# microsoft/DirectXTex

Measured on AMD Instinct MI355X. Metric: Mtexels/s BC7 encode (4096^2 RGBA8, TEX_COMPRESS_DEFAULT), higher is better.
Workload: dtype fp32 seed fit + i32 exact error sums (u8 texels in, 128-bit blocks out); 1 GPU; cfg2: 4096x4096 RGBA8 -> BC7_UNORM, TEX_COMPRESS_DEFAULT, one image per GPU, source and payload resident in HBM (dxtex_compress_device)

## Files before the change

directxtex_amd/csrc/bc6h_encode.hip:

```cpp
#include "dxtex_kernels.h"
#include "bc67_tables.h"
#include "bc7_core.h"
#include "bc6h_core.h"
#include "search_common.h"
#include <algorithm>
#include <cstdlib>
#include <cstdio>
#include <vector>

namespace dxtex
{
namespace
{
using namespace bc6h;

struct Ep16 { uint32_t a01, a2b0, b12; };
__device__ __forceinline__ Ep16 pack_ep16(const int (&A)[3], const int (&B)[3])
{
    Ep16 e;
    e.a01 = (uint32_t(A[0]) & 0xFFFFu) | (uint32_t(A[1]) << 16);
    e.a2b0 = (uint32_t(A[2]) & 0xFFFFu) | (uint32_t(B[0]) << 16);
    e.b12 = (uint32_t(B[1]) & 0xFFFFu) | (uint32_t(B[2]) << 16);
    return e;
}
// ... 1043 lines not shown
}

hipError_t launch_bc6h_encode(const SrcView& src, uint8_t* dst, uint64_t dstRowPitch, bool isSigned, void* scratch,
                              hipStream_t stream, KernelMarks* marks, const SideStreams* side)
{
    BcImage one; one.src = src; one.dst = dst; one.dstRowPitch = dstRowPitch;
    return launch_bc6h_encode_many(&one, 1, isSigned, scratch, stream, marks, side);
}

hipError_t launch_bc6h_encode_many(const BcImage* images, size_t count, bool isSigned, void* scratch, hipStream_t stream, KernelMarks* marks,
                                   const SideStreams* side)
{
#define DXTEX_MARK(NAME) do { if (marks) marks->mark(NAME); } while (0)
    std::vector<BcSeg> segs;
    std::vector<BcPass> passes;
    uint64_t perPass = 0;
    if (!build_passes(images, count, kMaxBlocksPerPass6, segs, passes, &perPass)) return hipSuccess;
    const Scratch6 L(perPass);
    uint8_t* base = static_cast<uint8_t*>(scratch);
    BcSeg* dSegs = reinterpret_cast<BcSeg*>(base + L.total);
    const hipError_t ce = upload_segments(dSegs, segs, passes, stream);
    if (ce != hipSuccess) return ce;
    for (const BcPass& pass : passes)
    {
        Bc6hArgs a;
        set_pass(a.seg, dSegs, segs, pass);
        a.nblocks = pass.nblocks;
        a.isSigned = isSigned ? 1 : 0;
        static const bool noPrune = dev_env("DXTEX_BC6H_NO_PRUNE") != nullptr;
        a.prune = noPrune ? 0 : 1;
        a.fpix = reinterpret_cast<float*>(base + L.fpix);
        a.lists = base + L.lists;
        a.seeds = reinterpret_cast<int*>(base + L.seeds);
        a.recs = reinterpret_cast<Rec6*>(base + L.recs);
        a.orgs = reinterpret_cast<OrgSave*>(base + L.orgs);
        a.order = reinterpret_cast<uint2*>(base + L.order);
        a.tinfo = reinterpret_cast<uint32_t*>(base + L.tinfo);
        a.counters = reinterpret_cast<uint32_t*>(base + L.counters);
        a.best = reinterpret_cast<Best6*>(base + L.best);
        a.bounds = reinterpret_cast<float*>(base + L.bounds);
        a.opts = reinterpret_cast<OptSave*>(base + L.opts);
        a.saveOpt = 0;
        a.boundsReady = 0;
        a.filterStats = 0;
        a.mode = ModeRt();

        DXTEX_MARK("bc6h_rough");
        hipLaunchKernelGGL(bc6h_rough_kernel, dim3((a.nblocks + 3) / 4), dim3(256), 0, stream, a);
        DXTEX_MARK("bc6h_block_seed");
        hipLaunchKernelGGL(bc6h_block_seed_kernel, dim3((a.nblocks + 255) / 256), dim3(256), 0, stream, a);
        if (dev_env("DXTEX_BC6H_DUMP"))
        {
            (void)hipStreamSynchronize(stream);
            const uint32_t n = std::min<uint32_t>(a.nblocks, 4);
            std::vector<uint8_t> l(n * 8); std::vector<int> sd(n * SEED_INTS);
            (void)hipMemcpy(l.data(), a.lists, l.size(), hipMemcpyDeviceToHost);
            (void)hipMemcpy(sd.data(), a.seeds, sd.size() * 4, hipMemcpyDeviceToHost);
            for (uint32_t b = 0; b < n; ++b)
            {
                fprintf(stderr, "block %u shapes:", b);
                for (int i = 0; i < 8; ++i) fprintf(stderr, " %d", l[b * 8 + i]);
                fprintf(stderr, "\n  seeds rank0:");
                for (int i = 0; i < 12; ++i) fprintf(stderr, " %d", sd[b * SEED_INTS + i]);
                fprintf(stderr, "\n");
            }
        }
        static const int onlyMode = dev_env("DXTEX_BC6H_ONLY_MODE") ? atoi(dev_env("DXTEX_BC6H_ONLY_MODE")) : -1;
        static const bool noSearch = dev_env("DXTEX_BC6H_NO_SEARCH") != nullptr;
        static const Bc6hMode kModes[14] = {
            { 0x00, 1, 1, 3, { 10, 10, 10 }, { 5, 5, 5 } }, { 0x01, 1, 1, 3, { 7, 7, 7 }, { 6, 6, 6 } }, { 0x02, 1, 1, 3, { 11, 11, 11 }, { 5, 4, 4 } },
            { 0x06, 1, 1, 3, { 11, 11, 11 }, { 4, 5, 4 } }, { 0x0a, 1, 1, 3, { 11, 11, 11 }, { 4, 4, 5 } }, { 0x0e, 1, 1, 3, { 9, 9, 9 }, { 5, 5, 5 } },
            { 0x12, 1, 1, 3, { 8, 8, 8 }, { 6, 5, 5 } }, { 0x16, 1, 1, 3, { 8, 8, 8 }, { 5, 6, 5 } }, { 0x1a, 1, 1, 3, { 8, 8, 8 }, { 5, 5, 6 } },
            { 0x1e, 1, 0, 3, { 6, 6, 6 }, { 6, 6, 6 } }, { 0x03, 0, 0, 4, { 10, 10, 10 }, { 10, 10, 10 } }, { 0x07, 0, 1, 4, { 11, 11, 11 }, { 9, 9, 9 } },
            { 0x0b, 0, 1, 4, { 12, 12, 12 }, { 8, 8, 8 } }, { 0x0f, 0, 1, 4, { 16, 16, 16 }, { 4, 4, 4 } } };
        auto set_mode_on = [&](Bc6hArgs& a, int mi)
        {
            const Bc6hMode& k = kModes[mi];
            a.mode.index = mi; a.mode.code = k.code; a.mode.regions2 = k.regions2; a.mode.transformed = k.transformed; a.mode.prec = k.prec[0];
            for (int c = 0; c < 3; ++c) a.mode.delta[c] = k.delta[c];
        };
        auto set_mode = [&](int mi) { set_mode_on(a, mi); };
        auto sort_tasks = [&](const Bc6hArgs& a, uint32_t ntasks, hipStream_t stream)
        {
            const uint32_t binGroups = std::min<uint32_t>(kBinGroups, (ntasks + 255) / 256);
            (void)hipMemsetAsync(a.counters, 0, 128 * sizeof(uint32_t), stream);
            hipLaunchKernelGGL(bc7_bin_count_kernel, dim3(binGroups), dim3(256), 0, stream, a.tinfo, ntasks, a.counters);
            hipLaunchKernelGGL(bc7_bin_scan_kernel, dim3(1), dim3(1), 0, stream, a.counters);
            hipLaunchKernelGGL(bc7_bin_scatter_kernel, dim3(binGroups), dim3(256), 0, stream, a.tinfo, ntasks, a.counters, a.order);
        };
        a.taskBase = 0;
        for (int m = 0; m < 4; ++m) a.prec1[m] = kModes[10 + m].prec[0];
        static const std::vector<int> order6 = []
        {
            std::vector<int> o;
            const char* e = dev_env("DXTEX_BC6H_ORDER");
            const char* p = e ? e : DXTEX_BC6H_DEFAULT_ORDER;
            while (*p) { if (*p >= '0' && *p <= '9') o.push_back(int(strtol(p, const_cast<char**>(&p), 10))); else ++p; }
            return o;
        }();
        int prevPrec = -1;
        a.samePrec = 0;
        std::vector<int> run2;
        for (int mi : order6) if (mi >= 0 && mi <= 9 && (onlyMode < 0 || mi == onlyMode)) run2.push_back(mi);
        static const int forkBack = dev_env("DXTEX_BC6H_FORK_BACK") ? atoi(dev_env("DXTEX_BC6H_FORK_BACK")) : 2;
        const SideStreams* fork = (marks || forkBack <= 0 || run2.size() < size_t(forkBack) + 1 || onlyMode >= 0) ? nullptr : side;
        Bc6hArgs a1 = a;
        a1.recs = reinterpret_cast<Rec6*>(base + L.recs1);
        a1.orgs = reinterpret_cast<OrgSave*>(base + L.orgs1);
        a1.order = reinterpret_cast<uint2*>(base + L.order1);
        a1.tinfo = reinterpret_cast<uint32_t*>(base + L.tinfo1);
        a1.counters = reinterpret_cast<uint32_t*>(base + L.counters1);
        a1.samePrec = 0;
        auto one_region_search = [&](hipStream_t stream, KernelMarks* marks)
        {
            const uint32_t gridPP = (a1.nblocks + 255) / 256;
            DXTEX_MARK("bc6h_pre_1region");
            a1.boundsReady = 0;
            for (int m = 0; m < 4; ++m)
            {
                if (onlyMode >= 0 && 10 + m != onlyMode) continue;
                set_mode_on(a1, 10 + m); a1.taskBase = uint32_t(m) * a1.nblocks;
                hipLaunchKernelGGL(bc6h_pre_kernel<0>, dim3(gridPP), dim3(256), 0, stream, a1);
                a1.boundsReady = 1;
            }
            const uint32_t ntasks = a1.nblocks * 4u;
            if (onlyMode >= 0)
                for (int m = 0; m < 4; ++m) if (10 + m != onlyMode) (void)hipMemsetAsync(a1.tinfo + uint64_t(m) * a1.nblocks, 0, uint64_t(a1.nblocks) * 4, stream);
            DXTEX_MARK("bc6h_bin_1region");
            sort_tasks(a1, ntasks, stream);
            DXTEX_MARK("bc6h_perturb_1region");
            static const uint32_t waveMax = dev_env("DXTEX_BC6H_WAVE_MAX") ? uint32_t(strtoul(dev_env("DXTEX_BC6H_WAVE_MAX"), nullptr, 0)) : kWaveTaskMax6;
            if (!noSearch)
            {
                hipLaunchKernelGGL(bc6h_perturb_kernel<16>, dim3(std::min<uint32_t>(kSearchWaves, (ntasks + 63) / 64)), dim3(64), 0, stream, a1, waveMax);
                hipLaunchKernelGGL(bc6h_perturb_wave_kernel, dim3(std::min<uint32_t>(kSearchWaves, ntasks)), dim3(64), 0, stream, a1, waveMax);
            }
        };
        bool forked = false;
        for (size_t at = 0; at < run2.size(); ++at)
        {
            const int mi = run2[at];
            if (fork && at + size_t(forkBack) == run2.size())
            {
                (void)hipEventRecord(fork->forked, stream);
                (void)hipStreamWaitEvent(fork->side[0], fork->forked, 0);
                one_region_search(fork->side[0], nullptr);
                (void)hipEventRecord(fork->joined[0], fork->side[0]);
                forked = true;
            }
            set_mode(mi);
            static const bool noReuse = dev_env("DXTEX_BC6H_NO_REUSE") != nullptr;
            a.samePrec = (!noReuse && prevPrec == kModes[mi].prec[0]) ? 1 : 0;
            prevPrec = kModes[mi].prec[0];
            a.saveOpt = (!noReuse && at + 1 < run2.size() && kModes[run2[at + 1]].prec[0] == kModes[mi].prec[0]) ? 1 : 0;
            const uint32_t ntasks = a.nblocks * 16u;
            const uint32_t gridPP = (a.nblocks + 15) / 16;
            static const char* const kPre[10] = { "bc6h_pre_m0", "bc6h_pre_m1", "bc6h_pre_m2", "bc6h_pre_m3", "bc6h_pre_m4", "bc6h_pre_m5", "bc6h_pre_m6", "bc6h_pre_m7", "bc6h_pre_m8", "bc6h_pre_m9" };
            static const char* const kPerturb[10] = { "bc6h_perturb_m0", "bc6h_perturb_m1", "bc6h_perturb_m2", "bc6h_perturb_m3", "bc6h_perturb_m4", "bc6h_perturb_m5", "bc6h_perturb_m6", "bc6h_perturb_m7", "bc6h_perturb_m8", "bc6h_perturb_m9" };
            static const char* const kPost[10] = { "bc6h_post_m0", "bc6h_post_m1", "bc6h_post_m2", "bc6h_post_m3", "bc6h_post_m4", "bc6h_post_m5", "bc6h_post_m6", "bc6h_post_m7", "bc6h_post_m8", "bc6h_post_m9" };
            DXTEX_MARK(kPre[mi]);
            hipLaunchKernelGGL(bc6h_pre_kernel<1>, dim3(gridPP), dim3(256), 0, stream, a);
            a.boundsReady = 1;
            DXTEX_MARK("bc6h_bin_2region");
            sort_tasks(a, ntasks, stream);
#if defined(DXTEX_DEV)
            static const bool stats6 = dev_env("DXTEX_BC6H_STATS") != nullptr;
            a.filterStats = stats6 ? 1 : 0;
            if (stats6)
            {
                uint32_t c[40] = {};
                (void)hipStreamSynchronize(stream);
// ... 57 lines not shown
```

directxtex_amd/csrc/bc7_encode.hip:

```cpp
#include "dxtex_kernels.h"
#include "bc67_tables.h"
#include "bc7_core.h"
#include "search_common.h"
#include <algorithm>
#include <cstdio>
#include <cstdlib>
#include <vector>

namespace dxtex
{
namespace
{
using namespace bc7;

struct Cand { uint32_t err; uint32_t ord; uint64_t lo, hi; };

enum : int { SLOT_M0 = 0, SLOT_M1, SLOT_M2, SLOT_M3, SLOT_M4A, SLOT_M4B, SLOT_M5, SLOT_M6, SLOT_M7, NUM_SLOTS };
enum : int { LIST_BYTES = 64 };

enum : int { PHASE_ALL = 0, PHASE_EARLY = 1, PHASE_LATE = 2 };

struct Bc7Args
{
    SegTable seg;
// ... 308 lines not shown
    if (a.gate && *a.gate < a.gateMin) return;
    const uint32_t blk = uint32_t(lane) / TM::TPB, r = uint32_t(lane) % TM::TPB;
    const uint32_t nb = nbFirst + blk;
    uint32_t shape, mask, anchor, rot;
    const bool active = (blk < uint32_t(BPW)) && task_geometry<MODE, IM>(a, nb, r, shape, mask, anchor, rot);
    TaskRec rec; rec.A = 0; rec.B = 0; rec.err = 0; rec.orgErr = 0;
    uint32_t npLive = 0;
    if (!__any(active))
    {
        if (nb < a.nblocks && blk < uint32_t(BPW))
        {
            a.recs[uint64_t(nb) * TM::TPB + r] = rec;
            a.tinfo[uint64_t(nb) * TM::TPB + r] = 0;
        }
        return;
    }
    stage_packed<BPW>(a, nbFirst, lane, sL[wave]);
    int lb = 0;
    if (active)
    {
        SubsetResult res; int np; Region rg; Block16 b16;
        task_org<MODE, IM>(nullptr, &sL[wave][blk * 16], mask, anchor, rot, res, np, true, rg, b16,
                           (TM::NS == 2) ? a.seeds + uint64_t(nb) * 64 + (TM::LIST ? 32 : 0) + r
                                         : (TM::NS == 1) ? a.seeds1 + uint64_t(nb) * 2 : a.seeds3 + uint64_t(nb) * 192 + shape * 3 + (r % TM::G));
        rec.A = res.orgA; rec.B = res.orgB; rec.err = res.orgErr; rec.orgErr = res.orgErr;
        npLive = (res.orgErr != 0) ? uint32_t(np) : 0u;
        if (a.prune && npLive)
        {
            lb = subset_lower_bound(&sL[wave][blk * 16], mask, rot, (MODE >= 6) ? 4 : 3);
            if (MODE == 4 || MODE == 5)
            {
                if (rot != 0 || lst_has_alpha(a, nb))
                    lb += scalar_kmeans_lower_bound<(MODE == 4 && IM == 0) ? 8 : 4>(&sL[wave][blk * 16], rot);
            }
            if (MODE < 4)
            {
                const uint32_t* pix = &sL[wave][blk * 16];
#pragma unroll
                for (int i = 0; i < 16; ++i) if ((mask >> i) & 1u) { const int da = 255 - int(pix[i] >> 24); lb += da * da; }
            }
        }
    }
    if (a.prune)
    {
        int candOrg = active ? rec.err : 0, candLb = lb;
#pragma unroll
        for (int d = 1; d < TM::G; d <<= 1) { candOrg += __shfl_xor(candOrg, d); candLb += __shfl_xor(candLb, d); }
        int table = active ? candOrg : 0x7FFFFFFF;
#pragma unroll
        for (int d = TM::G; d < TM::TPB && d < 64; d <<= 1) table = min(table, __shfl_xor(table, d));
        if (nb < a.nblocks && blk < uint32_t(BPW)) table = min(table, a.bestErr[nb]);
        if (candLb > table) npLive = 0;
    }
    if (nb < a.nblocks && blk < uint32_t(BPW))
    {
        a.recs[uint64_t(nb) * TM::TPB + r] = rec;
        a.tinfo[uint64_t(nb) * TM::TPB + r] = (mask & 0xFFFFu) | (rot << 16) | (npLive << 24);
    }
}

template<int MODE, int IM>
__device__ __forceinline__ void search_pickup(const Bc7Args& a, uint2 task, uint32_t* slotCol, SlotRegion& rg)
{
    typedef TaskMap<MODE, IM> TM;
    const uint32_t nb = task.x / TM::TPB;
    const uint32_t mask = task.y & 0xFFFFu, rot = (task.y >> 16) & 3u;
    const uint4* px4 = reinterpret_cast<const uint4*>(a.px + uint64_t(nb) * 16);
    const uint4 q0 = px4[0], q1 = px4[1], q2 = px4[2], q3 = px4[3];
    const uint32_t px[16] = { q0.x, q0.y, q0.z, q0.w, q1.x, q1.y, q1.z, q1.w, q2.x, q2.y, q2.z, q2.w, q3.x, q3.y, q3.z, q3.w };
    int np = 0;
    if (TM::NS == 1)
    {
#pragma unroll
        for (int i = 0; i < 16; ++i) slotCol[i * kSlotStride] = rotate_pixel(px[i], rot);
        np = 16;
    }
    else
    {
#pragma unroll
        for (int i = 0; i < 16; ++i)
            if ((mask >> i) & 1u) { slotCol[np * kSlotStride] = px[i]; ++np; }
    }
    rg.base = slotCol; rg.np = np; rg.p2sum = 0;
}

__device__ __forceinline__ int lanes_below(unsigned long long mask)
{
    return int(__builtin_amdgcn_mbcnt_hi(uint32_t(mask >> 32), __builtin_amdgcn_mbcnt_lo(uint32_t(mask), 0u)));
}

#if defined(DXTEX_BC7_WAVETIMES)
enum : int { WT_KINDS = 3, WT_KEYS = WT_KINDS * 8 * 2 * 3, WT_FIELDS = 6 };
__device__ unsigned long long g_wt[WT_KEYS][8192][WT_FIELDS];
__device__ unsigned int g_wtHist[WT_KEYS][256];
#define WT_BEGIN(KIND) const int wtKey = (((KIND) * 8 + MODE) * 2 + IM) * 3 + CHSET; const bool wtOn = a.phase != PHASE_EARLY; \
    const unsigned long long wt0 = wall_clock64(); unsigned long long wtDr = 0, wtRounds = 0, wtLanes = 0, wtTasks = 0; int wtMine = 0
#define WT_TAKE(IDX) do { wtTasks += (unsigned long long)__popcll(__ballot((IDX) != 0xFFFFFFFFu)); if (!wtDr && q.drained) wtDr = wall_clock64(); } while (0)
#define WT_ROUND(BUSYL) do { ++wtRounds; wtLanes += (unsigned long long)__popcll(__ballot(BUSYL)); if (BUSYL) ++wtMine; } while (0)
#define WT_DONE() do { wtMine = 0; } while (0)
#define WT_END() do { if (wtOn && lane == 0 && wtRounds) { unsigned long long* w_ = g_wt[wtKey][blockIdx.x & 8191]; w_[0] = wt0; w_[1] = wtDr ? wtDr : wall_clock64(); \
    w_[2] = wall_clock64(); w_[3] = wtRounds; w_[4] = wtLanes; w_[5] = wtTasks; } } while (0)
#else
#define WT_BEGIN(KIND) do { } while (0)
#define WT_TAKE(IDX) do { } while (0)
#define WT_ROUND(BUSYL) do { } while (0)
#define WT_DONE() do { } while (0)
#define WT_END() do { } while (0)
#endif
#if !defined(DXTEX_FLAT_SKIP)
#define DXTEX_FLAT_SKIP 1
#endif
template<int MODE, int IM, int CHSET>
constexpr bool kFlatSkip = DXTEX_FLAT_SKIP != 0 && MODE == 6 && CHSET == CH_ALL;

template<int MODE, int IM, int CHSET>
__global__ void __launch_bounds__(64) bc7_perturb_kernel(Bc7Args a, int loop)
{
    typedef LoopCfg<MODE, IM, CHSET> C;
    __shared__ uint32_t sSlot[16 * kSlotStride];
    const int lane = threadIdx.x;
    const uint32_t live = a.counters[34];
    if (live == 0) return;
    if (TaskMap<MODE, IM>::NS == 1 && live <= a.perturbWaveMax) return;
    uint32_t* head = a.counters + kQueueBase + loop;
    uint32_t* slotCol = &sSlot[lane];
    WT_BEGIN(0);

    PerturbState st = perturb_begin<MODE, IM, CHSET>(0, 0, 0);
    SlotRegion rg; rg.base = slotCol; rg.np = 0; rg.p2sum = 0;
    int base = 0;
    uint32_t myTask = 0xFFFFFFFFu;
    uint32_t flatMask = 0, flatVals = 0;
    WaveQueue q; q.lo = q.hi = 0; q.drained = false;
    for (;;)
    {
        const unsigned long long idle = __ballot(myTask == 0xFFFFFFFFu);
        if (idle && !(q.drained && q.lo >= q.hi))
        {
            const uint32_t idx = queue_take(q, head, live, idle, lane);
            WT_TAKE(idx);
            if (idx != 0xFFFFFFFFu)
            {
                const uint2 task = a.order[idx];
                myTask = task.x;
                const TaskRec r = a.recs[myTask];
                search_pickup<MODE, IM>(a, task, slotCol, rg);
                st = perturb_begin<MODE, IM, CHSET>(r.A, r.B, r.err);
                int other;
                base = loop_base<MODE, IM, CHSET>(rg, st.optA, st.optB, &other);
                if (loop_is_settled<CHSET>(r.err, other)) myTask = 0xFFFFFFFFu;
                if constexpr (kFlatSkip<MODE, IM, CHSET>) flatMask = flat_channels(rg, flatVals);
            }
        }
        if constexpr (kFlatSkip<MODE, IM, CHSET>)
        {
            const bool fc = myTask != 0xFFFFFFFFu && flat_call<MODE, IM, CHSET>(st, flatMask, flatVals);
            if (__any(fc))
            {
                const int nearest = eval_nearest<MODE, IM, CHSET>(rg, st, base);
                if (fc && nearest == st.optErr)
                {
                    st = skip_flat_calls<MODE, IM, CHSET>(st);
                    if (st.ch >= C::CH1)
                    {
                        TaskRec* r = a.recs + myTask;
                        r->A = st.optA; r->B = st.optB; r->err = st.optErr;
                        myTask = 0xFFFFFFFFu;
                        WT_DONE();
                    }
                }
            }
// ... 777 lines not shown
    uint64_t lo = 0, hi = 0;
#pragma unroll
    for (int s = 0; s < NUM_SLOTS; ++s)
    {
        if (!((slotMask >> s) & 1u)) continue;
        if (s == SLOT_M7 && a.flagged[1] == 0) continue;
        const Cand v = c[s];
        if (v.err == 0xFFFFFFFFu) continue;
        const uint64_t key = (uint64_t(v.err) << 32) | v.ord;
        if (key < bestKey) { bestKey = key; lo = v.lo; hi = v.hi; }
    }
    const BcSeg& sg = seg_of(a.seg, nb);
    const uint32_t gb = sg.nb0 + (nb - sg.l0);
    const uint32_t by = gb / sg.nbw, bx = gb - by * sg.nbw;
    uint64_t* out = reinterpret_cast<uint64_t*>(sg.dst + uint64_t(by) * sg.dstRowPitch) + 2 * uint64_t(bx);
    out[0] = lo; out[1] = hi;
}
}

namespace
{
const uint64_t kMaxBlocksPerPass = dev_env("DXTEX_MAX_BLOCKS_PER_PASS") ? std::max<uint64_t>(1, strtoull(dev_env("DXTEX_MAX_BLOCKS_PER_PASS"), nullptr, 10)) : (1u << 22);
constexpr int kMaxTasksPerBlock = 64;
const uint64_t kSmallPassBlocks = dev_env("DXTEX_BC7_SMALL_BLOCKS") ? strtoull(dev_env("DXTEX_BC7_SMALL_BLOCKS"), nullptr, 10) : 262144;
struct ScratchLayout
{
    size_t lists, cands, px, recs, order, tinfo, counters, zeroOrd, bestErr, seeds, seeds1, seeds3, flagcnt, auxRecs, auxOrder, auxTinfo, auxCounters, total;
    size_t auxTpb, auxSlices;
    explicit ScratchLayout(uint64_t nb, bool threeSubsets)
    {
        auto up = [](size_t v) { return (v + 255) & ~size_t(255); };
        const size_t tpb = threeSubsets ? kMaxTasksPerBlock : 32;
        const bool small = nb <= kSmallPassBlocks;
        auxTpb = small ? tpb : 4; auxSlices = small ? size_t(kSideStreams) : 2;
        size_t o = 0;
        lists = o; o = up(o + nb * LIST_BYTES);
        cands = o; o = up(o + nb * NUM_SLOTS * sizeof(Cand));
        px = o; o = up(o + nb * 64);
        recs = o; o = up(o + nb * tpb * sizeof(TaskRec));
        order = o; o = up(o + nb * tpb * sizeof(uint2));
        tinfo = o; o = up(o + nb * tpb * sizeof(uint32_t));
        counters = o; o = up(o + 64 * sizeof(uint32_t));
        zeroOrd = o; o = up(o + nb * sizeof(uint32_t));
        bestErr = o; o = up(o + nb * sizeof(int));
        seeds = o; o = up(o + nb * 64 * sizeof(uint2));
        seeds1 = o; o = up(o + nb * 2 * sizeof(uint2));
        seeds3 = o; o = up(o + (threeSubsets ? nb * 192 * sizeof(uint2) : 0));
        flagcnt = o; o = up(o + 256);
        auxRecs = o; o = up(o + auxSlices * nb * auxTpb * sizeof(TaskRec));
        auxOrder = o; o = up(o + auxSlices * nb * auxTpb * sizeof(uint2));
        auxTinfo = o; o = up(o + auxSlices * nb * auxTpb * sizeof(uint32_t));
        auxCounters = o; o = up(o + size_t(kSideStreams) * 64 * sizeof(uint32_t));
        total = o;
    }
};

template<int MODE, int IM>
void launch_mode(const Bc7Args& a0, hipStream_t stream, KernelMarks* marks, const char* const (&names)[7])
{
    typedef TaskMap<MODE, IM> TM;
    constexpr int BPW = (TM::TPB >= 64) ? 1 : 64 / TM::TPB;
    const uint32_t nb = a0.nblocks;
    const uint32_t ntasks = nb * uint32_t(TM::TPB);
    const uint32_t gridPP = (nb + 4 * BPW - 1) / (4 * BPW);
    constexpr bool kWhole = TM::NS == 1;
    constexpr uint32_t kExhMax = (MODE == 6) ? kWaveTaskMax : kWaveTaskMax45;
    static const bool noGroup = dev_env("DXTEX_BC7_NO_GROUP") != nullptr;
    const bool maybeShortP = kWhole && !noGroup && (MODE == 6 || ntasks <= 4u * kPerturbWaveMax);
    const bool maybeShortE = kWhole && !noGroup && (MODE == 6 || ntasks <= 4u * kExhMax);
    const uint32_t wavesP = std::min<uint32_t>(kSearchWaves, (ntasks + 1) / 2), wavesE = std::min<uint32_t>(kSearchWaves, ntasks);
    Bc7Args a = a0;
    a.gate = nullptr; a.gateMin = 0;
    if (a0.flagged && !(a0.flags & BCF_BC7_QUICK))
    {
        if (MODE == 7) { a.gate = a0.flagged + 1; a.gateMin = 1; }
        else if (a0.phase == PHASE_EARLY && (MODE == 4 || MODE == 5)) { a.gate = a0.flagged + 1; a.gateMin = std::max<uint32_t>(1u, a0.earlyAlphaMin); }
        else if (a0.phase == PHASE_EARLY && MODE == 6) { a.gate = a0.flagged; a.gateMin = std::max<uint32_t>(1u, a0.early6Min); }
    }
    a.perturbWaveMax = maybeShortP ? kPerturbWaveMax : 0u;
    a.exhWaveMax = maybeShortE ? kExhMax : 0u;
    if (marks) marks->mark(names[0]);
    hipLaunchKernelGGL((bc7_pre_kernel<MODE, IM>), dim3(gridPP), dim3(256), 0, stream, a);
    if (marks) marks->mark(names[1]);
    (void)hipMemsetAsync(a.counters, 0, 64 * sizeof(uint32_t), stream);
    const uint32_t binGroups = std::min<uint32_t>(kBinGroups, (ntasks + 255) / 256);
    hipLaunchKernelGGL(bc7_bin_count_kernel, dim3(binGroups), dim3(256), 0, stream, a.tinfo, ntasks, a.counters, a.gate, a.gateMin);
    hipLaunchKernelGGL(bc7_bin_scan_kernel, dim3(1), dim3(1), 0, stream, a.counters);
    hipLaunchKernelGGL(bc7_bin_scatter_kernel, dim3(binGroups), dim3(256), 0, stream, a.tinfo, ntasks, a.counters, a.order, a.gate, a.gateMin);
    if (marks) marks->mark(names[2]);
    const uint32_t waves = std::min<uint32_t>(kSearchWaves, (ntasks + 63) / 64);
    static const int tailBelow = dev_env("DXTEX_BC7_TAIL_BELOW") ? atoi(dev_env("DXTEX_BC7_TAIL_BELOW")) : 48;
    static const bool perturbPlain = dev_env("DXTEX_BC7_PERTURB_PLAIN") != nullptr;
    static const int rangeTests = dev_env("DXTEX_BC7_NO_PEEL") ? 3 : ((dev_env("DXTEX_BC7_RANGE_TESTS") ? atoi(dev_env("DXTEX_BC7_RANGE_TESTS")) & 0xFF : DXTEX_RANGE_TESTS) |
                                                                       ((dev_env("DXTEX_BC7_PEEL_LAYERS") ? atoi(dev_env("DXTEX_BC7_PEEL_LAYERS")) : 1) << 8));
    if constexpr (PaletteBits<MODE, IM>::AB == 0)
    {
        if constexpr (MODE == 1 || MODE == 6)
        {
            if (perturbPlain) hipLaunchKernelGGL((bc7_perturb_kernel<MODE, IM, CH_ALL>), dim3(waves), dim3(64), 0, stream, a, 0);
            else hipLaunchKernelGGL((bc7_perturb_filter_kernel<MODE, IM, CH_ALL>), dim3(waves), dim3(64), 0, stream, a, 0);
        }
        else
            hipLaunchKernelGGL((bc7_perturb_kernel<MODE, IM, CH_ALL>), dim3(waves), dim3(64), 0, stream, a, 0);
        if constexpr (kWhole) { if (maybeShortP) hipLaunchKernelGGL((bc7_perturb_wave_kernel<MODE, IM, CH_ALL>), dim3(wavesP), dim3(64), 0, stream, a); }
        if (marks) marks->mark(names[4]);
        if constexpr (kWhole) { if (maybeShortE) hipLaunchKernelGGL((bc7_exhaustive_wave_kernel<MODE, IM, CH_ALL>), dim3(wavesE), dim3(64), 0, stream, a); }
        hipLaunchKernelGGL((bc7_exhaustive_kernel<MODE, IM, CH_ALL>), dim3(waves), dim3(64), 0, stream, a, 1, tailBelow, rangeTests);
    }
    else
    {
        if constexpr (MODE == 4 && IM == 1 && DXTEX_PF_M4 != 0)
        {
            if (perturbPlain) hipLaunchKernelGGL((bc7_perturb_kernel<MODE, IM, CH_COLOR>), dim3(waves), dim3(64), 0, stream, a, 0);
            else hipLaunchKernelGGL((bc7_perturb_filter_kernel<MODE, IM, CH_COLOR>), dim3(waves), dim3(64), 0, stream, a, 0);
        }
        else
            hipLaunchKernelGGL((bc7_perturb_kernel<MODE, IM, CH_COLOR>), dim3(waves), dim3(64), 0, stream, a, 0);
        if (maybeShortP) hipLaunchKernelGGL((bc7_perturb_wave_kernel<MODE, IM, CH_COLOR>), dim3(wavesP), dim3(64), 0, stream, a);
        if (marks) marks->mark(names[3]);
        hipLaunchKernelGGL((bc7_perturb_kernel<MODE, IM, CH_ALPHA>), dim3(waves), dim3(64), 0, stream, a, 1);
        if (maybeShortP) hipLaunchKernelGGL((bc7_perturb_wave_kernel<MODE, IM, CH_ALPHA>), dim3(wavesP), dim3(64), 0, stream, a);
        if (marks) marks->mark(names[4]);
        if (maybeShortE) hipLaunchKernelGGL((bc7_exhaustive_wave_kernel<MODE, IM, CH_COLOR>), dim3(wavesE), dim3(64), 0, stream, a);
        hipLaunchKernelGGL((bc7_exhaustive_kernel<MODE, IM, CH_COLOR>), dim3(waves), dim3(64), 0, stream, a, 2, tailBelow, rangeTests);
        if (marks) marks->mark(names[5]);
        if (maybeShortE) hipLaunchKernelGGL((bc7_exhaustive_wave_kernel<MODE, IM, CH_ALPHA>), dim3(wavesE), dim3(64), 0, stream, a);
        hipLaunchKernelGGL((bc7_exhaustive_kernel<MODE, IM, CH_ALPHA>), dim3(waves), dim3(64), 0, stream, a, 3, tailBelow, rangeTests);
    }
    if (marks) marks->mark(names[6]);
    hipLaunchKernelGGL((bc7_post_kernel<MODE, IM>), dim3(gridPP), dim3(256), 0, stream, a);
#if defined(DXTEX_DEV)
    static const bool stats = dev_env("DXTEX_BC7_STATS") != nullptr;
    if (stats)
    {
        uint32_t c[40] = {};
        (void)hipStreamSynchronize(stream);
        (void)hipMemcpy(c, a.counters, sizeof(c), hipMemcpyDeviceToHost);
        std::fprintf(stderr, "bc7 stats %-22s phase %d: %9u task slots, %9u live; by size 16..1:", names[0], a.phase, ntasks, c[34]);
        for (int b = 16; b >= 1; --b) std::fprintf(stderr, " %u", c[b]);
        std::fprintf(stderr, "\n");
    }
#endif
}
}

#if defined(DXTEX_BC7_WAVETIMES)
namespace
{
void bc7_wavetimes_report()
{
    (void)hipDeviceSynchronize();
    static int call = 0;
    static const int wanted = dev_env("DXTEX_BC7_WT_CALL") ? atoi(dev_env("DXTEX_BC7_WT_CALL")) : 2;
    const bool print = call++ == wanted;
    static std::vector<unsigned long long> h(size_t(WT_KEYS) * 8192 * WT_FIELDS);
    static std::vector<unsigned int> hist(size_t(WT_KEYS) * 256);
    (void)hipMemcpyFromSymbol(h.data(), HIP_SYMBOL(g_wt), h.size() * 8);
    (void)hipMemcpyFromSymbol(hist.data(), HIP_SYMBOL(g_wtHist), hist.size() * 4);
    unsigned long long tAll = ~0ull;
    for (size_t i = 0; i < size_t(WT_KEYS) * 8192; ++i) if (h[i * WT_FIELDS + 2]) tAll = std::min(tAll, h[i * WT_FIELDS]);
    static const char* const kinds[3] = { "perturb", "perturb_filter", "exhaustive" };
    for (int key = 0; key < WT_KEYS; ++key)
    {
        const unsigned long long* w = h.data() + size_t(key) * 8192 * WT_FIELDS;
        std::vector<unsigned long long> st, dr, en; unsigned long long rounds = 0, lanes = 0, life = 0, maxR = 0, tasks = 0, maxT = 0;
        for (int i = 0; i < 8192; ++i)
            if (w[i * WT_FIELDS + 2])
            {
                st.push_back(w[i * WT_FIELDS]); dr.push_back(w[i * WT_FIELDS + 1]); en.push_back(w[i * WT_FIELDS + 2]);
                rounds += w[i * WT_FIELDS + 3]; lanes += w[i * WT_FIELDS + 4]; tasks += w[i * WT_FIELDS + 5];
                life += w[i * WT_FIELDS + 2] - w[i * WT_FIELDS]; maxR = std::max(maxR, w[i * WT_FIELDS + 3]); maxT = std::max(maxT, w[i * WT_FIELDS + 5]);
// ... 246 lines not shown
```

directxtex_amd/csrc/search_common.h:

```cpp
#pragma once
#include <hip/hip_runtime.h>
#include <stdint.h>
#include <algorithm>
#include <cstring>
#include <vector>
#include "dxtex_kernels.h"

namespace dxtex
{
namespace
{
struct BcSeg
{
    SrcView src;
    uint8_t* dst;
    uint64_t dstRowPitch;
    uint32_t nbw;
    uint32_t nb0;
    uint32_t l0;
    uint32_t pad;
};

struct SegTable
{
// ... 40 lines not shown

inline hipError_t upload_segments(BcSeg* dSegs, std::vector<BcSeg>& segs, const std::vector<BcPass>& passes, hipStream_t stream)
{
    bool needTable = false;
    for (const BcPass& pass : passes) needTable |= pass.nseg > 2;
    if (!needTable) return hipSuccess;
    struct Staging { void* host = nullptr; size_t capacity = 0; hipEvent_t consumed = nullptr; bool pending = false; int device = -1; };
    static thread_local Staging st;
    int device = 0;
    hipError_t e = hipGetDevice(&device);
    if (e != hipSuccess) return e;
    if (st.pending) { e = hipEventSynchronize(st.consumed); if (e != hipSuccess) return e; st.pending = false; }
    const size_t bytes = segs.size() * sizeof(BcSeg);
    if (st.device != device || st.capacity < bytes)
    {
        if (st.host) (void)hipHostFree(st.host);
        if (st.consumed) (void)hipEventDestroy(st.consumed);
        st = Staging();
        e = hipHostMalloc(&st.host, std::max<size_t>(bytes, 4096), hipHostMallocDefault);
        if (e != hipSuccess) return e;
        e = hipEventCreateWithFlags(&st.consumed, hipEventDisableTiming);
        if (e != hipSuccess) return e;
        st.capacity = std::max<size_t>(bytes, 4096); st.device = device;
    }
    std::memcpy(st.host, segs.data(), bytes);
    e = hipMemcpyAsync(dSegs, st.host, bytes, hipMemcpyHostToDevice, stream);
    if (e != hipSuccess) return e;
    e = hipEventRecord(st.consumed, stream);
    st.pending = (e == hipSuccess);
    return e;
}

inline void set_pass(SegTable& t, const BcSeg* dSegs, const std::vector<BcSeg>& segs, const BcPass& pass)
{
    t.segs = dSegs + pass.seg0; t.nseg = pass.nseg;
    t.inl[0] = segs[pass.seg0]; t.inl[1] = segs[pass.seg0 + (pass.nseg > 1 ? 1 : 0)];
}

inline size_t seg_table_bytes(uint64_t nblocks, uint64_t maxPerPass, size_t nimages)
{
    const uint64_t perPass = nblocks < maxPerPass ? nblocks : maxPerPass;
    const uint64_t passes = perPass ? (nblocks + perPass - 1) / perPass : 1;
    return ((nimages + passes + 1) * sizeof(BcSeg) + 255) & ~size_t(255);
}

__device__ __forceinline__ void wave_lds_sync()
{
    __builtin_amdgcn_fence(__ATOMIC_RELEASE, "wavefront");
    __builtin_amdgcn_wave_barrier();
    __builtin_amdgcn_fence(__ATOMIC_ACQUIRE, "wavefront");
}

__device__ __forceinline__ int wave_prefix_min(int v)
{
    v = min(v, __builtin_amdgcn_update_dpp(v, v, 0x111, 0xF, 0xF, false));
    v = min(v, __builtin_amdgcn_update_dpp(v, v, 0x112, 0xF, 0xF, false));
    v = min(v, __builtin_amdgcn_update_dpp(v, v, 0x114, 0xF, 0xF, false));
    v = min(v, __builtin_amdgcn_update_dpp(v, v, 0x118, 0xF, 0xF, false));
    v = min(v, __builtin_amdgcn_update_dpp(v, v, 0x142, 0xA, 0xF, false));
    v = min(v, __builtin_amdgcn_update_dpp(v, v, 0x143, 0xC, 0xF, false));
    return v;
}

__device__ __forceinline__ void selection_pass(int& e, uint32_t& s, int lane, int i)
{
    const int v = (lane >= i) ? e : 0x7FFFFFFF;
    const int incl = wave_prefix_min(v);
    int excl = __builtin_amdgcn_update_dpp(0x7FFFFFFF, incl, 0x138, 0xF, 0xF, false);
    if (lane <= i) excl = 0x7FFFFFFF;
    const bool isrec = (lane > i) && (e < excl);
    const unsigned long long mask = __ballot(isrec);
    int srcLane = lane;
    if (isrec)
    {
        const unsigned long long below = mask & ((1ull << lane) - 1ull);
        srcLane = below ? (63 - __clzll(below)) : i;
    }
    else if (lane == i && mask)
        srcLane = 63 - __clzll(mask);
    e = __shfl(e, srcLane);
    s = uint32_t(__shfl(int(s), srcLane));
}

constexpr int kBinGroups = 2048;

__global__ void __launch_bounds__(256) bc7_bin_count_kernel(const uint32_t* tinfo, uint32_t ntasks, uint32_t* counters, const uint32_t* gate = nullptr, uint32_t gateMin = 0)
{
    if (gate && *gate < gateMin) return;
    __shared__ uint32_t hist[17];
    if (threadIdx.x < 17) hist[threadIdx.x] = 0;
    __syncthreads();
    const uint32_t per = (ntasks + gridDim.x - 1) / gridDim.x;
    const uint32_t t0 = blockIdx.x * per, t1 = min(ntasks, t0 + per);
    for (uint32_t t = t0 + threadIdx.x; t < t1; t += 256)
    {
        const uint32_t np = tinfo[t] >> 24;
        if (np) atomicAdd(&hist[np], 1u);
    }
    __syncthreads();
    if (threadIdx.x >= 1 && threadIdx.x <= 16 && hist[threadIdx.x]) atomicAdd(&counters[threadIdx.x], hist[threadIdx.x]);
}

__global__ void bc7_bin_scan_kernel(uint32_t* counters)
{
    if (threadIdx.x != 0 || blockIdx.x != 0) return;
    uint32_t run = 0;
    for (int b = 16; b >= 1; --b) { counters[17 + b] = run; run += counters[b]; }
    counters[34] = run;
}

__global__ void __launch_bounds__(256) bc7_bin_scatter_kernel(const uint32_t* tinfo, uint32_t ntasks, uint32_t* counters, uint2* order, const uint32_t* gate = nullptr, uint32_t gateMin = 0)
{
    if (gate && *gate < gateMin) return;
    __shared__ uint32_t hist[17], cursor[17];
    if (threadIdx.x < 17) hist[threadIdx.x] = 0;
    __syncthreads();
    const uint32_t per = (ntasks + gridDim.x - 1) / gridDim.x;
    const uint32_t t0 = blockIdx.x * per, t1 = min(ntasks, t0 + per);
    for (uint32_t t = t0 + threadIdx.x; t < t1; t += 256)
    {
        const uint32_t np = tinfo[t] >> 24;
        if (np) atomicAdd(&hist[np], 1u);
    }
    __syncthreads();
    if (threadIdx.x >= 1 && threadIdx.x <= 16)
        cursor[threadIdx.x] = hist[threadIdx.x] ? atomicAdd(&counters[17 + threadIdx.x], hist[threadIdx.x]) : 0u;
    __syncthreads();
    for (uint32_t t = t0 + threadIdx.x; t < t1; t += 256)
    {
        const uint32_t ti = tinfo[t], np = ti >> 24;
        if (np) order[atomicAdd(&cursor[np], 1u)] = make_uint2(t, ti);
    }
}

constexpr int kQueueBase = 36;
constexpr int kSearchWaves = 8192;

constexpr uint32_t kQueueBatch = 128;

struct WaveQueue
{
    uint32_t lo, hi;
    bool drained;
};

__device__ __forceinline__ uint32_t queue_take(WaveQueue& q, uint32_t* head, uint32_t live, unsigned long long idle, int lane)
{
    if (q.lo >= q.hi && !q.drained)
    {
        const uint32_t batch = (live > uint32_t(kSearchWaves) * 64u) ? kQueueBatch : 64u;
        uint32_t base = 0;
        if (lane == 0) base = atomicAdd(head, batch);
        base = uint32_t(__builtin_amdgcn_readfirstlane(int(base)));
        q.lo = base;
        q.hi = min(base + batch, live);
        if (base >= live) { q.drained = true; q.hi = q.lo; }
    }
    const uint32_t k = uint32_t(__popcll(idle & ((1ull << lane) - 1ull)));
    const uint32_t avail = q.hi - q.lo;
    const uint32_t mine = (((idle >> lane) & 1ull) && k < avail) ? (q.lo + k) : 0xFFFFFFFFu;
    q.lo += min(uint32_t(__popcll(idle)), avail);
    return mine;
}

}
}
```

Measured before the change: 136.5 Mtexels/s.

## Replace LDS-atomic task binning with wave-ballot stable counting sort

```diff
diff --git a/directxtex_amd/csrc/bc6h_encode.hip b/directxtex_amd/csrc/bc6h_encode.hip
--- a/directxtex_amd/csrc/bc6h_encode.hip
+++ b/directxtex_amd/csrc/bc6h_encode.hip
@@ -1149,11 +1149,7 @@
         auto set_mode = [&](int mi) { set_mode_on(a, mi); };
         auto sort_tasks = [&](const Bc6hArgs& a, uint32_t ntasks, hipStream_t stream)
         {
-            const uint32_t binGroups = std::min<uint32_t>(kBinGroups, (ntasks + 255) / 256);
-            (void)hipMemsetAsync(a.counters, 0, 128 * sizeof(uint32_t), stream);
-            hipLaunchKernelGGL(bc7_bin_count_kernel, dim3(binGroups), dim3(256), 0, stream, a.tinfo, ntasks, a.counters);
-            hipLaunchKernelGGL(bc7_bin_scan_kernel, dim3(1), dim3(1), 0, stream, a.counters);
-            hipLaunchKernelGGL(bc7_bin_scatter_kernel, dim3(binGroups), dim3(256), 0, stream, a.tinfo, ntasks, a.counters, a.order);
+            launch_task_sort(a.tinfo, ntasks, a.counters, 128, a.order, nullptr, 0, stream);
         };
         a.taskBase = 0;
         for (int m = 0; m < 4; ++m) a.prec1[m] = kModes[10 + m].prec[0];
diff --git a/directxtex_amd/csrc/bc7_encode.hip b/directxtex_amd/csrc/bc7_encode.hip
--- a/directxtex_amd/csrc/bc7_encode.hip
+++ b/directxtex_amd/csrc/bc7_encode.hip
@@ -414,11 +414,6 @@
             if ((mask >> i) & 1u) { slotCol[np * kSlotStride] = px[i]; ++np; }
     }
     rg.base = slotCol; rg.np = np; rg.p2sum = 0;
-}
-
-__device__ __forceinline__ int lanes_below(unsigned long long mask)
-{
-    return int(__builtin_amdgcn_mbcnt_hi(uint32_t(mask >> 32), __builtin_amdgcn_mbcnt_lo(uint32_t(mask), 0u)));
 }
 
 #if defined(DXTEX_BC7_WAVETIMES)
@@ -1362,11 +1357,7 @@
     if (marks) marks->mark(names[0]);
     hipLaunchKernelGGL((bc7_pre_kernel<MODE, IM>), dim3(gridPP), dim3(256), 0, stream, a);
     if (marks) marks->mark(names[1]);
-    (void)hipMemsetAsync(a.counters, 0, 64 * sizeof(uint32_t), stream);
-    const uint32_t binGroups = std::min<uint32_t>(kBinGroups, (ntasks + 255) / 256);
-    hipLaunchKernelGGL(bc7_bin_count_kernel, dim3(binGroups), dim3(256), 0, stream, a.tinfo, ntasks, a.counters, a.gate, a.gateMin);
-    hipLaunchKernelGGL(bc7_bin_scan_kernel, dim3(1), dim3(1), 0, stream, a.counters);
-    hipLaunchKernelGGL(bc7_bin_scatter_kernel, dim3(binGroups), dim3(256), 0, stream, a.tinfo, ntasks, a.counters, a.order, a.gate, a.gateMin);
+    launch_task_sort(a.tinfo, ntasks, a.counters, 64, a.order, a.gate, a.gateMin, stream);
     if (marks) marks->mark(names[2]);
     const uint32_t waves = std::min<uint32_t>(kSearchWaves, (ntasks + 63) / 64);
     static const int tailBelow = dev_env("DXTEX_BC7_TAIL_BELOW") ? atoi(dev_env("DXTEX_BC7_TAIL_BELOW")) : 48;
diff --git a/directxtex_amd/csrc/search_common.h b/directxtex_amd/csrc/search_common.h
--- a/directxtex_amd/csrc/search_common.h
+++ b/directxtex_amd/csrc/search_common.h
@@ -146,23 +146,88 @@
     s = uint32_t(__shfl(int(s), srcLane));
 }
 
+__device__ __forceinline__ int lanes_below(unsigned long long mask)
+{
+    return int(__builtin_amdgcn_mbcnt_hi(uint32_t(mask >> 32), __builtin_amdgcn_mbcnt_lo(uint32_t(mask), 0u)));
+}
+
 constexpr int kBinGroups = 2048;
 
+__device__ __forceinline__ void bin_wave_part(uint32_t ntasks, uint32_t& w0, uint32_t& w1)
+{
+    const uint32_t per = ((ntasks + gridDim.x - 1) / gridDim.x + 255u) & ~255u;
+    const uint32_t wave = uint32_t(__builtin_amdgcn_readfirstlane(int(threadIdx.x >> 6)));
+    const uint64_t at = uint64_t(blockIdx.x) * per + uint64_t(wave) * (per / 4);
+    w0 = at < ntasks ? uint32_t(at) : ntasks;
+    w1 = at + per / 4 < ntasks ? uint32_t(at + per / 4) : ntasks;
+}
+
+template<bool PLACE>
+__device__ __forceinline__ uint32_t bin_wave_walk(const uint32_t* tinfo, uint32_t w0, uint32_t w1, uint32_t run, uint2* order)
+{
+    const uint32_t lane = threadIdx.x & 63u;
+    const bool aligned = (reinterpret_cast<uintptr_t>(tinfo) & 15u) == 0;
+    for (uint32_t c = w0; c < w1; c += 256)
+    {
+        const uint32_t t = c + 4u * lane;
+        uint32_t ti[4] = { 0u, 0u, 0u, 0u };
+        if (aligned && t + 4u <= w1)
+        {
+            const uint4 q = *reinterpret_cast<const uint4*>(tinfo + t);
+            ti[0] = q.x; ti[1] = q.y; ti[2] = q.z; ti[3] = q.w;
+        }
+        else
+        {
+#pragma unroll
+            for (int k = 0; k < 4; ++k) if (t + k < w1) ti[k] = tinfo[t + k];
+        }
+        uint32_t slot[4] = { 0u, 0u, 0u, 0u };
+        uint32_t pending = 0;
+#pragma unroll
+        for (int k = 0; k < 4; ++k) if (ti[k] >> 24) pending |= 1u << ((ti[k] >> 24) & 31u);
+        for (unsigned long long todo = __ballot(pending != 0); todo; todo = __ballot(pending != 0))
+        {
+            const uint32_t size = uint32_t(__ffs(__builtin_amdgcn_readlane(int(pending), __ffsll(todo) - 1)) - 1);
+            uint32_t below = 0, total = 0;
+#pragma unroll
+            for (int k = 0; k < 4; ++k)
+            {
+                const unsigned long long same = __ballot((ti[k] >> 24) == size);
+                below += uint32_t(lanes_below(same));
+                total += uint32_t(__popcll(same));
+            }
+            if (PLACE)
+            {
+                uint32_t at = uint32_t(__builtin_amdgcn_readlane(int(run), int(size))) + below;
+#pragma unroll
+                for (int k = 0; k < 4; ++k) if ((ti[k] >> 24) == size) slot[k] = at++;
+            }
+            if (lane == size) run += total;
+            pending &= ~(1u << size);
+        }
+        if (PLACE)
+        {
+#pragma unroll
+            for (int k = 0; k < 4; ++k) if (ti[k] >> 24) order[slot[k]] = make_uint2(t + k, ti[k]);
+        }
+    }
+    return run;
+}
+
 __global__ void __launch_bounds__(256) bc7_bin_count_kernel(const uint32_t* tinfo, uint32_t ntasks, uint32_t* counters, const uint32_t* gate = nullptr, uint32_t gateMin = 0)
 {
     if (gate && *gate < gateMin) return;
-    __shared__ uint32_t hist[17];
-    if (threadIdx.x < 17) hist[threadIdx.x] = 0;
+    __shared__ uint32_t whist[4][17];
+    uint32_t w0, w1;
+    bin_wave_part(ntasks, w0, w1);
+    const uint32_t lane = threadIdx.x & 63u, cnt = bin_wave_walk<false>(tinfo, w0, w1, 0u, nullptr);
+    if (lane >= 1 && lane <= 16) whist[threadIdx.x >> 6][lane] = cnt;
     __syncthreads();
-    const uint32_t per = (ntasks + gridDim.x - 1) / gridDim.x;
-    const uint32_t t0 = blockIdx.x * per, t1 = min(ntasks, t0 + per);
-    for (uint32_t t = t0 + threadIdx.x; t < t1; t += 256)
-    {
-        const uint32_t np = tinfo[t] >> 24;
-        if (np) atomicAdd(&hist[np], 1u);
-    }
-    __syncthreads();
-    if (threadIdx.x >= 1 && threadIdx.x <= 16 && hist[threadIdx.x]) atomicAdd(&counters[threadIdx.x], hist[threadIdx.x]);
+    if (threadIdx.x >= 1 && threadIdx.x <= 16)
+    {
+        const uint32_t total = whist[0][threadIdx.x] + whist[1][threadIdx.x] + whist[2][threadIdx.x] + whist[3][threadIdx.x];
+        if (total) atomicAdd(&counters[threadIdx.x], total);
+    }
 }
 
 __global__ void bc7_bin_scan_kernel(uint32_t* counters)
@@ -176,25 +241,34 @@
 __global__ void __launch_bounds__(256) bc7_bin_scatter_kernel(const uint32_t* tinfo, uint32_t ntasks, uint32_t* counters, uint2* order, const uint32_t* gate = nullptr, uint32_t gateMin = 0)
 {
     if (gate && *gate < gateMin) return;
-    __shared__ uint32_t hist[17], cursor[17];
-    if (threadIdx.x < 17) hist[threadIdx.x] = 0;
-    __syncthreads();
-    const uint32_t per = (ntasks + gridDim.x - 1) / gridDim.x;
-    const uint32_t t0 = blockIdx.x * per, t1 = min(ntasks, t0 + per);
-    for (uint32_t t = t0 + threadIdx.x; t < t1; t += 256)
-    {
-        const uint32_t np = tinfo[t] >> 24;
-        if (np) atomicAdd(&hist[np], 1u);
-    }
+    __shared__ uint32_t whist[4][17], base[17];
+    uint32_t w0, w1;
+    bin_wave_part(ntasks, w0, w1);
+    const uint32_t lane = threadIdx.x & 63u, wave = threadIdx.x >> 6, cnt = bin_wave_walk<false>(tinfo, w0, w1, 0u, nullptr);
+    if (lane >= 1 && lane <= 16) whist[wave][lane] = cnt;
     __syncthreads();
     if (threadIdx.x >= 1 && threadIdx.x <= 16)
-        cursor[threadIdx.x] = hist[threadIdx.x] ? atomicAdd(&counters[17 + threadIdx.x], hist[threadIdx.x]) : 0u;
+    {
+        const uint32_t total = whist[0][threadIdx.x] + whist[1][threadIdx.x] + whist[2][threadIdx.x] + whist[3][threadIdx.x];
+        base[threadIdx.x] = total ? atomicAdd(&counters[17 + threadIdx.x], total) : 0u;
+    }
     __syncthreads();
-    for (uint32_t t = t0 + threadIdx.x; t < t1; t += 256)
-    {
-        const uint32_t ti = tinfo[t], np = ti >> 24;
-        if (np) order[atomicAdd(&cursor[np], 1u)] = make_uint2(t, ti);
-    }
+    uint32_t cursor = 0;
+    if (lane >= 1 && lane <= 16)
+    {
+        cursor = base[lane];
+        for (uint32_t w = 0; w < wave; ++w) cursor += whist[w][lane];
+    }
+    bin_wave_walk<true>(tinfo, w0, w1, cursor, order);
+}
+
+inline void launch_task_sort(const uint32_t* tinfo, uint32_t ntasks, uint32_t* counters, uint32_t counterWords, uint2* order, const uint32_t* gate, uint32_t gateMin, hipStream_t stream)
+{
+    (void)hipMemsetAsync(counters, 0, counterWords * sizeof(uint32_t), stream);
+    const uint32_t binGroups = std::min<uint32_t>(kBinGroups, (ntasks + 255) / 256);
+    hipLaunchKernelGGL(bc7_bin_count_kernel, dim3(binGroups), dim3(256), 0, stream, tinfo, ntasks, counters, gate, gateMin);
+    hipLaunchKernelGGL(bc7_bin_scan_kernel, dim3(1), dim3(1), 0, stream, counters);
+    hipLaunchKernelGGL(bc7_bin_scatter_kernel, dim3(binGroups), dim3(256), 0, stream, tinfo, ntasks, counters, order, gate, gateMin);
 }
 
 constexpr int kQueueBase = 36;
```

New measurement: 136.6 Mtexels/s (median of 2 runs). No clear change (+0.1%).
